# benfred/implicit

Hardware: AMD Instinct MI355X
Metric: ALS user+item updates/sec per iteration (factors=128); top-k recs/sec (higher is better)
Workload: dtype f32; 1 GPU; BASELINE configs[2]: last.fm-360K-shaped synthetic CSR, ALS CG cg_steps=3; users=358868, items=292385, nnz=17308340, factors=128, solver=cg, cg_steps=3

## Files before the change

### implicit_amd/csrc/als_cg_q.hip

```cpp
#include <type_traits>

#include "als_qtile.h"
#include "common.h"

namespace imp {

template <typename T>
void launch_team_fused(const imp_csr *C, int f, int width, int first, int count, T *X, const T *Y, const float *A0, int cg_steps,
                       const char *name);
template <typename T>
void launch_group_fused(const imp_csr *C, int f, int first, int count, T *X, const T *Y, const float *A0, int cg_steps, const char *name);
template <typename ST>
void launch_team_tile64(const imp_csr *C, int f, int width, int first, int count, ST *X, const ST *Y, const float *A0, int cg_steps,
                        const char *name);

template <int F, typename T> static void run_classes_q(const imp_csr *C, T *X, const T *Y, const float *A0, int cg_steps) {
  const int32_t *b = C->bin_start;
  constexpr bool kHalf = std::is_same<T, __half>::value;
  auto team = [&](int width32, int lo, int hi, const char *name) {
    if constexpr (kHalf) launch_team_tile64<T>(C, F, width32 / 2, lo, hi - lo, X, Y, A0, cg_steps, name);
    else launch_team_fused<T>(C, F, width32, lo, hi - lo, X, Y, A0, cg_steps, name);
  };
  team(16, b[1], b[2], "als_cg_team16_rows");
  team(8, b[2], b[3], "als_cg_team8_rows");
  team(4, b[3], b[4], "als_cg_team4_rows");
  team(2, b[4], b[5], "als_cg_team2_rows");
  if constexpr (F == 64) launch_team_fused<T>(C, F, 1, b[5], b[7] - b[5], X, Y, A0, cg_steps, "als_cg_short_rows");
  else launch_group_fused<T>(C, F, b[5], b[7] - b[5], X, Y, A0, cg_steps, "als_cg_short_rows");
}

template <typename T> void least_squares_cg_q(const imp_csr *C, T *X, const T *Y, const float *A0, int f, int cg_steps) {
  if (f == 128) run_classes_q<128, T>(C, X, Y, A0, cg_steps);
  else if (f == 64) run_classes_q<64, T>(C, X, Y, A0, cg_steps);
  else throw std::invalid_argument("least_squares_cg_q: f must be 64 or 128");
}
template void least_squares_cg_q<float>(const imp_csr *, float *, const float *, const float *, int, int);
template void least_squares_cg_q<__half>(const imp_csr *, __half *, const __half *, const float *, int, int);

}
```

### implicit_amd/csrc/als_cg_qf.hip

```cpp
#include <type_traits>

#include "als_qf_common.h"
#include "common.h"

namespace imp {

template <typename ST> struct Tile32 {
  typedef f32x2 elem;
  static constexpr int T = 32;
  static constexpr bool ROLL = std::is_same<ST, float>::value;
  static __device__ __forceinline__ void fetch(const int32_t *indices, const float *data, int lane, int k0, int end, int &col, float &c) {
    fetch_entries(indices, data, lane, k0, end, col, c);
  }
  template <int H> static __device__ __forceinline__ void gather(elem (&yq)[H], const ST *p) {
#pragma unroll
    for (int h = 0; h < H; h += 2) {
      const float4 v = load4(p + 32 * h);
      yq[h] = f32x2{v.x, v.y}, yq[h + 1] = f32x2{v.z, v.w};
    }
  }
  template <int H> static __device__ __forceinline__ float dot(const elem (&yq)[H], const f32x2 (&ve)[H]) {
    f32x2 s = yq[0] * ve[0];
#pragma unroll
    for (int h = 1; h < H; ++h) s = __builtin_elementwise_fma(yq[h], ve[h], s);
    return s.x + s.y;
  }
  template <int H> static __device__ __forceinline__ void axpy(const elem (&yq)[H], float w, f32x2 (&ae)[H]) {
    const f32x2 w2 = {w, w};
#pragma unroll
    for (int h = 0; h < H; ++h) ae[h] = __builtin_elementwise_fma(w2, yq[h], ae[h]);
  }
};

template <int F, int WPR, int BLOCK, typename ST>
__global__ __launch_bounds__(BLOCK, F == 64 ? 8 : 4) void als_cg_qfteam_kernel(const int32_t *__restrict__ order, int first, int count,
                                                                 const int32_t *__restrict__ indptr,
                                                                 const int32_t *__restrict__ indices,
                                                                 const float *__restrict__ data, ST *__restrict__ X,
                                                                 const ST *__restrict__ Y, const float *__restrict__ A0,
                                                                 int cg_steps) {
  team_rows<Tile32<ST>, F, WPR, BLOCK>(order, first, count, indptr, indices, data, X, Y, A0, cg_steps);
}

template <int F, int WPR, int BLOCK, typename T>
static void launch_qfteam(const imp_csr *C, int first, int count, T *X, const T *Y, const float *A0, int cg_steps,
                          const char *name) {
  if (count <= 0) return;
  constexpr int WAVES = BLOCK / 64, TEAMS = WAVES / WPR;
  size_t lds = team_lds_bytes<F, WPR, BLOCK, Tile32<T>::T>();
  auto kern = als_cg_qfteam_kernel<F, WPR, BLOCK, T>;
  IMP_CHECK_HIP(hipFuncSetAttribute(reinterpret_cast<const void *>(kern), hipFuncAttributeMaxDynamicSharedMemorySize, (int)lds));
  int per_cu = (int)std::max<size_t>(1, std::min<size_t>(2048 / BLOCK, (160 * 1024) / lds));
  constexpr int kBaseOversub = WPR <= 4 ? 4 : (WPR == 8 ? 2 : (F == 64 ? 2 : 1));
  int grid = std::min((count + TEAMS - 1) / TEAMS, ctx().num_cus * per_cu * std::max(kBaseOversub, ctx().oversub));
  IMP_PROF(name);
  kern<<<grid, BLOCK, lds, stream()>>>(C->order.data(), first, count, C->indptr.data(), C->indices.data(), C->data.data(), X, Y,
                                      A0, cg_steps);
  IMP_CHECK_HIP(hipGetLastError());
}

typedef float f32x4 __attribute__((ext_vector_type(4)));
template <int F> struct QFGroupCfg {
  static constexpr int LD = F + 8;
  static constexpr int LDB = F + 8;
  static constexpr int NT = F / 16;
  static constexpr int KH = 16 / NT;
  static constexpr int KB = (F / 16) / KH;
  static constexpr size_t lds_bytes = (size_t)3 * F * LDB * 2 + (size_t)3 * 16 * LDB * 2 +
                                      ((size_t)16 * LD + (size_t)KH * 16 * LD + 16 * 64) * sizeof(float);
};
typedef __bf16 bf16x8 __attribute__((ext_vector_type(8)));
typedef __bf16 bf16x2 __attribute__((ext_vector_type(2)));
__device__ __forceinline__ void split_bf16(float x, __bf16 &hi, __bf16 &mid, __bf16 &lo) {
  hi = (__bf16)x;
  const float r1 = x - (float)hi;
  mid = (__bf16)r1;
  lo = (__bf16)(r1 - (float)mid);
}

template <int F, bool FIRST, bool LAST, bool ROLL, typename ST>
__device__ __forceinline__ float tile_pass(f32x2 (&y)[8][F / 32], float *cw, int cnt, const float *vrow, float (&acc)[F / 64], int lane,
                                          int cnt_nx, int &col_nx, float &c_nx, const ST *__restrict__ Y) {
  using Tile = Tile32<ST>;
  constexpr int FE = F / 16, H = FE / 2;
  static_assert(!(FIRST && LAST) && (LAST || !ROLL), "pass form");
  if constexpr (ROLL) {
    col_nx = opaque(col_nx);
    c_nx = __int_as_float(opaque(__float_as_int(c_nx)));
  }
  f32x2 ve[H], ae[H];
  const float *cwg;
  {
// ... 295 lines not shown
```

### implicit_amd/csrc/als_qf_common.h

```cpp
#ifndef IMPLICIT_AMD_CSRC_ALS_QF_COMMON_H_
#define IMPLICIT_AMD_CSRC_ALS_QF_COMMON_H_
#include <type_traits>
#include <utility>

#include "als_qtile.h"

namespace imp {

__device__ __forceinline__ int opaque(int v) {
  asm volatile("" : "+v"(v));
  return v;
}

typedef float f32x2 __attribute__((ext_vector_type(2)));

template <int I> using idx_t = std::integral_constant<int, I>;
template <int N, typename Fn, int... Is> __device__ __forceinline__ void static_for_impl(Fn &&fn, std::integer_sequence<int, Is...>) {
  (fn(idx_t<Is>{}), ...);
}
template <int N, typename Fn> __device__ __forceinline__ void static_for(Fn &&fn) {
  static_for_impl<N>(fn, std::make_integer_sequence<int, N>{});
}

template <int F, int NJ, int TICKS> struct DenseTicks {
// ... 8 lines not shown
      if constexpr (NJ == 1) vj2 = f32x2{vp[0], 0.f};
      else if constexpr (s % 2 == 0) vj2 = *reinterpret_cast<const f32x2 *>(vp + s);
#pragma unroll
      for (int e = 0; e < Q4; ++e) a[e] = *reinterpret_cast<const float4 *>(row + (size_t)s * F + 64 * e);
    }
  }
  template <int K> __device__ __forceinline__ void consume(f32x2 (&ae)[FE / 2]) {
    if constexpr (K % EVERY == 0) {
      constexpr int s = K / EVERY;
      const float vj = (s % 2 == 0) ? vj2.x : vj2.y;
      const f32x2 v2 = {vj, vj};
#pragma unroll
      for (int e = 0; e < Q4; ++e) {
        ae[2 * e] = __builtin_elementwise_fma(v2, f32x2{a[e].x, a[e].y}, ae[2 * e]);
        ae[2 * e + 1] = __builtin_elementwise_fma(v2, f32x2{a[e].z, a[e].w}, ae[2 * e + 1]);
      }
    }
  }
};

__device__ __forceinline__ float reduce_pair(float d0, float d1) {
  float u = d1 + dpp_mov<0x128>(d1);
  const float s0 = d0 + dpp_mov<0x128>(d0);
  u = __builtin_bit_cast(float, __builtin_amdgcn_update_dpp(__builtin_bit_cast(int, u), __builtin_bit_cast(int, s0), 0xE4, 0xF, 0x3,
                                                            false));
  u += dpp_mov<0x141>(u);
  u += dpp_mov<0xB1>(u);
  u += dpp_mov<0x4E>(u);
  return u;
}
template <int LANE> __device__ __forceinline__ float row_bcast_from(float v) {
  return dpp_mov<0x150 + LANE>(v);
}

enum : unsigned { kGo = 1u, kLast = 2u };

#ifndef IMP_TEAM_NAP_FIRST
#define IMP_TEAM_NAP_FIRST 6
#endif
#ifndef IMP_TEAM_NAP_NEXT
#define IMP_TEAM_NAP_NEXT 2
#endif
#ifndef IMP_TEAM_NAP_LEADER
#define IMP_TEAM_NAP_LEADER 1
#endif
#ifndef IMP_TEAM_LEADER_PRIO
#define IMP_TEAM_LEADER_PRIO 0
#endif


template <typename Tile, int F, int P, typename ST>
__device__ __forceinline__ void gather_pair(typename Tile::elem (&y)[Tile::T / 4][F / 32], float *cw, int col_reg, float c_reg, int cnt,
                                            const ST *__restrict__ Y, int lane) {
  lane = opaque(lane);
  if ((lane >> 3) == P) {
    const bool ok = lane < cnt;
    cw[lane] = ok ? fabsf(c_reg) - 1.f : 0.f;
    cw[Tile::T + lane] = ok ? fmaxf(c_reg, 0.f) : 0.f;
  }
  const int src = 4 * (lane >> 4);
#pragma unroll
  for (int q = 2 * P; q < 2 * P + 2; ++q) {
    const unsigned col = (unsigned)__builtin_amdgcn_ds_bpermute(src + 16 * q, col_reg);
    Tile::template gather<F / 32>(y[q], Y + (size_t)col * F + 4 * (lane & 15));
  }
}
// ... 81 lines not shown
        dt.template issue<K>(row, vp);
        __builtin_amdgcn_sched_barrier(0);
        dt.template consume<K>(ae);
      });
    }
    if constexpr (ROLL) {
      if (8 * P < cnt_nx) gather_pair<Tile, F, P>(y, cw, col_nx, c_nx, cnt_nx, Y, lane);
    }
    __builtin_amdgcn_sched_barrier(0);
  });
  float pAp = 0.f;
  if constexpr (LAST) {
    f32x2 t = ae[0] * ve[0];
#pragma unroll
    for (int h = 1; h < H; ++h) t = __builtin_elementwise_fma(ae[h], ve[h], t);
    pAp = wave_allsum(fmaf(0.125f, s8, t.x + t.y));
  } else {
    float aes[FE];
#pragma unroll
    for (int h = 0; h < H; ++h) aes[2 * h] = ae[h].x, aes[2 * h + 1] = ae[h].y;
    reduce_expanded<F>(aes, acc);
  }
  if constexpr (ROLL) {
    Tile::fetch(indices, data, opaque(lane), k0_nx2, end_nx2, col_nx, c_nx);
  }
  return pAp;
}

template <int F, int WPR, int BLOCK, int T> constexpr size_t team_lds_bytes() {
  constexpr size_t WAVES = BLOCK / 64, TEAMS = WAVES / WPR;
  return ((size_t)F * F + WAVES * F + TEAMS * F + 2 * T * WAVES + 4 * TEAMS) * sizeof(float);
}

template <typename Tile, int F, int WPR, int BLOCK, typename ST>
__device__ __forceinline__ void team_rows(const int32_t *__restrict__ order, int first, int count, const int32_t *__restrict__ indptr,
                                          const int32_t *__restrict__ indices, const float *__restrict__ data, ST *__restrict__ X,
                                          const ST *__restrict__ Y, const float *__restrict__ A0, int cg_steps) {
  constexpr int FC = F / 64, FE = F / 16, T = Tile::T, WAVES = BLOCK / 64, TEAMS = WAVES / WPR, NJ = F / WPR / 4;
  static_assert(WPR <= WAVES && (F / WPR) % 4 == 0, "team width");
  extern __shared__ __attribute__((aligned(16))) float smem[];
  float *A0s = smem;
  float *parts = A0s + (size_t)F * F;
  float *vts = parts + (size_t)WAVES * F;
  float *cws = vts + (size_t)TEAMS * F;
  unsigned *ctl = reinterpret_cast<unsigned *>(cws + (size_t)WAVES * 2 * T);
  const int lane = threadIdx.x & 63;
  const int wave = __builtin_amdgcn_readfirstlane(threadIdx.x >> 6);
  const int team = wave / WPR, sub = wave % WPR;
  const bool leader = sub == 0;
  for (int e = threadIdx.x; e < F * F; e += BLOCK) A0s[e] = A0[e];
  if (threadIdx.x < 4 * TEAMS) ctl[threadIdx.x] = 0u;
  __syncthreads();
  const int j_begin = F * sub / WPR;
  float *vt = vts + (size_t)team * F;
  float *cw = cws + (size_t)wave * 2 * T;
  unsigned *arrivals = ctl + 4 * team, *generation = arrivals + 1, *words = arrivals + 2;

  unsigned gen = 0, pub = 0, arr_target = 0;
  auto lds_off = [](const void *ptr) { return (unsigned)(size_t)ptr; };
  const unsigned arrivals_off = lds_off(arrivals), generation_off = lds_off(generation), words_off = lds_off(words);
  const unsigned cf4 = 4u * (unsigned)QL<F>::cfactor(lane, 0);
  auto publish = [&](unsigned w) {
    ++pub;
    if (lane == 0)
      asm volatile("ds_write_b32 %0, %1\n\tds_add_u32 %2, %3" ::"v"(words_off + 4u * (pub & 1u)), "v"(w), "v"(generation_off), "v"(1u)
                   : "memory");
    if constexpr (IMP_TEAM_LEADER_PRIO > 0) __builtin_amdgcn_s_setprio(0);
  };
  auto poll = [&](unsigned off) {
    typedef __attribute__((address_space(3))) volatile unsigned lds_word;
    return (unsigned)__builtin_amdgcn_readfirstlane(*(lds_word *)(size_t)off);
  };
  auto await_operand = [&]() -> unsigned {
    ++gen;
    if constexpr (WPR > 1) {
      if (poll(generation_off) < gen) {
        __builtin_amdgcn_s_sleep(IMP_TEAM_NAP_FIRST);
        while (poll(generation_off) < gen) __builtin_amdgcn_s_sleep(IMP_TEAM_NAP_NEXT);
      }
    }
    return poll(words_off + 4u * (gen & 1u));
  };
  auto arrive = [&](const float (&acc)[FC]) {
// ... 31 lines not shown
    }
  };
  auto collect_scalar = [&](float own) -> float {
    arr_target += WPR;
    if constexpr (WPR > 1) {
      while (poll(arrivals_off) < arr_target) __builtin_amdgcn_s_sleep(IMP_TEAM_NAP_LEADER);
      asm volatile("" ::: "memory");
      if constexpr (IMP_TEAM_LEADER_PRIO > 0) __builtin_amdgcn_s_setprio(IMP_TEAM_LEADER_PRIO);
      const float *slot = parts + (size_t)(team * WPR) * F;
      float sum = 0.f;
#pragma unroll
      for (int w = 0; w < WPR; ++w) sum += slot[(size_t)w * F];
      return sum;
    } else {
      return own;
    }
  };
  auto operand_slot = [&]() { return reinterpret_cast<float *>(reinterpret_cast<char *>(vt) + cf4); };
  auto put_operand = [&](const float (&v)[FC]) {
    float *slot = operand_slot();
    if constexpr (FC == 2) *reinterpret_cast<float2 *>(slot) = make_float2(v[0], v[1]);
    else slot[0] = v[0];
  };
  auto get_operand = [&](float (&v)[FC]) {
    const float *slot = operand_slot();
    if constexpr (FC == 2) {
      const float2 t = *reinterpret_cast<const float2 *>(slot);
      v[0] = t.x, v[1] = t.y;
    } else {
      v[0] = slot[0];
    }
  };

  auto row_id = [&](int i) { return order[first + min(i, count - 1)]; };
  const int i_step = gridDim.x * TEAMS, i_first = blockIdx.x * TEAMS + team;
  auto slice = [&](int rb, int re, int &k0, int &cnt) {
    const int chunk = min(T, (((re - rb) + WPR - 1) / WPR + 3) & ~3);
    k0 = min(rb + chunk * sub, re);
    cnt = min(chunk, re - k0);
  };
  int id0 = row_id(i_first), id1 = row_id(i_first + i_step), id2 = row_id(i_first + 2 * i_step), id3 = row_id(i_first + 3 * i_step);
  int b0 = indptr[id0], e0 = indptr[id0 + 1], b1 = indptr[id1], e1 = indptr[id1 + 1], b2 = indptr[id2], e2 = indptr[id2 + 1];
  int ent_col, ent_cnt, k0;
  float ent_c;
  slice(b0, e0, k0, ent_cnt);
  Tile::fetch(indices, data, opaque(lane), k0, max(k0 + ent_cnt, b0 + 1), ent_col, ent_c);
  auto kill = [](float (&v)[FC]) {
#pragma unroll
    for (int cc = 0; cc < FC; ++cc) v[cc] = 0.f;
  };
  bool tile_ready = false;
  int cnt = 0;
  typename Tile::elem y[T / 4][FE / 2];
  float x[FC];
  kill(x);
  for (int i = i_first; i < count; i += i_step) {
    ST *xrow = X + (size_t)id0 * F;
    if (!tile_ready) {
      cnt = ent_cnt;
      ent_col = opaque(ent_col);
      ent_c = __int_as_float(opaque(__float_as_int(ent_c)));
      static_for<T / 8>([&](auto Pc) {
        constexpr int P = decltype(Pc)::value;
        if (8 * P < cnt) gather_pair<Tile, F, P>(y, cw, ent_col, ent_c, cnt, Y, lane);
      });
      slice(b1, e1, k0, ent_cnt);
      Tile::fetch(indices, data, opaque(lane), k0, max(k0 + ent_cnt, b1 + 1), ent_col, ent_c);
      if (leader) load_compact<F>(xrow, opaque(lane), x);
      else kill(x);
    }
    float xc[FC], r[FC], p[FC], Ap[FC], rsold = 0.f;
#pragma unroll
    for (int cc = 0; cc < FC; ++cc) xc[cc] = r[cc] = 0.f;
    bool store = false;
    if (leader) {
      put_operand(x);
#pragma unroll
      for (int cc = 0; cc < FC; ++cc) xc[cc] = x[cc];
      publish(kGo);
    }
    unsigned w = await_operand();
    {
      float acc[FC];
      fused_pass<Tile, F, NJ, true, false, false>(y, cw, cnt, vt, j_begin, A0s, acc, lane, 0, ent_col, ent_c, Y, nullptr, nullptr, 0, 0);
      arrive(acc);
    }
    if (leader) {
      collect(r);
#pragma unroll
      for (int cc = 0; cc < FC; ++cc) r[cc] = -r[cc], p[cc] = r[cc];
      rsold = dot_compact<F>(r, r);
      store = rsold >= 1e-20f;
      if (store && cg_steps > 0) {
        put_operand(p);
        publish(kGo | (cg_steps == 1 ? kLast : 0u));
      } else {
        publish(0u);
      }
    }
    w = await_operand();
    for (int it = 0; (w & (kGo | kLast)) == kGo; ++it) {
      float acc[FC];
      fused_pass<Tile, F, NJ, false, false, false>(y, cw, cnt, vt, j_begin, A0s, acc, lane, 0, ent_col, ent_c, Y, nullptr, nullptr, 0, 0);
      arrive(acc);
      if (leader) {
        collect(Ap);
        get_operand(p);
        const float alpha = rsold * __builtin_amdgcn_rcpf(dot_compact<F>(p, Ap));
#pragma unroll
        for (int cc = 0; cc < FC; ++cc) {
          xc[cc] = fmaf(alpha, p[cc], xc[cc]);
          r[cc] = fmaf(-alpha, Ap[cc], r[cc]);
        }
        const float rsnew = dot_compact<F>(r, r);
        if (rsnew < 1e-20f) {
          publish(0u);
        } else {
          const float beta = rsnew * __builtin_amdgcn_rcpf(rsold);
#pragma unroll
          for (int cc = 0; cc < FC; ++cc) p[cc] = fmaf(beta, p[cc], r[cc]);
          rsold = rsnew;
          put_operand(p);
          publish(kGo | (it + 2 >= cg_steps ? kLast : 0u));
        }
      }
      w = await_operand();
    }
    const bool rolled = Tile::ROLL && (w & kGo) != 0u;
    if (w & kGo) {
      float acc[FC], pAp;
      if constexpr (Tile::ROLL) {
        int k2, cnt2;
        slice(b2, e2, k2, cnt2);
        if (i + i_step >= count) ent_cnt = 0;
        pAp = fused_pass<Tile, F, NJ, false, true, true>(y, cw, cnt, vt, j_begin, A0s, acc, lane, ent_cnt, ent_col, ent_c, Y, indices,
                                                         data, k2, max(k2 + cnt2, b2 + 1));
        cnt = ent_cnt;
        ent_cnt = cnt2;
        if (leader) load_compact<F>(X + (size_t)id1 * F, opaque(lane), x);
        else kill(x);
      } else {
        kill(x);
        pAp = fused_pass<Tile, F, NJ, false, true, false>(y, cw, cnt, vt, j_begin, A0s, acc, lane, 0, ent_col, ent_c, Y, nullptr,
                                                          nullptr, 0, 0);
      }
      arrive_scalar(pAp);
      if (leader) {
        pAp = collect_scalar(pAp);
        get_operand(p);
        const float alpha = rsold * __builtin_amdgcn_rcpf(pAp);
#pragma unroll
        for (int cc = 0; cc < FC; ++cc) xc[cc] = fmaf(alpha, p[cc], xc[cc]);
        publish(0u);
      }
      (void)await_operand();
    } else {
      kill(x);
    }
    if (leader && store) store_compact<F>(xrow, opaque(lane), xc);
    tile_ready = rolled;
    id0 = id1, id1 = id2, id2 = id3, id3 = row_id(i + 4 * i_step);
    b0 = b1, e0 = e1, b1 = b2, e1 = e2, b2 = indptr[id2], e2 = indptr[id2 + 1];
  }
}

}
#endif
```

### implicit_amd/csrc/common.h

```cpp
#ifndef IMPLICIT_AMD_CSRC_COMMON_H_
#define IMPLICIT_AMD_CSRC_COMMON_H_

#include <hip/hip_runtime.h>

#include <climits>
#include <cstdint>
#include <cstdio>
#include <memory>
#include <mutex>
#include <stdexcept>
#include <string>
#include <vector>

#include "../../include/implicit_hip.h"
#include "csr_schedule.h"

namespace imp {

struct out_of_range_error : std::runtime_error {
  using std::runtime_error::runtime_error;
};

void set_last_error(const std::string &msg);

#define IMP_CHECK_HIP(expr)                                                                    \
  do {                                                                                         \
    hipError_t _e = (expr);                                                                    \
    if (_e != hipSuccess) {                                                                    \
      throw std::runtime_error(std::string("HIP error: ") + hipGetErrorString(_e) + " (" +    \
                               __FILE__ + ":" + std::to_string(__LINE__) + ")");             \
    }                                                                                          \
  } while (0)

struct Context;
Context &ctx();
std::unique_lock<std::recursive_mutex> lock_device();

template <typename F> int guarded(F &&body) {
  try {
    auto lock = lock_device();
    body();
    return IMP_OK;
  } catch (const std::invalid_argument &e) {
    set_last_error(e.what());
    return IMP_INVALID_ARGUMENT;
  } catch (const out_of_range_error &e) {
    set_last_error(e.what());
    return IMP_OUT_OF_RANGE;
// ... 15 lines not shown
    return IMP_INVALID_ARGUMENT;
  } catch (const out_of_range_error &e) {
    set_last_error(e.what());
    return IMP_OUT_OF_RANGE;
  } catch (const std::exception &e) {
    set_last_error(e.what());
    return IMP_RUNTIME_ERROR;
  } catch (...) {
    set_last_error("unknown error");
    return IMP_RUNTIME_ERROR;
  }
}

inline hipStream_t stream();
void sync();
void sync_call();
unsigned long long *fixup_total();
struct SolverSwitches {
  bool nm;
  bool w256;
  bool cg_pad;
  bool chol_nm;
  bool chol_pad;
};
const SolverSwitches &solver_switches();

struct ProfScope {
  explicit ProfScope(const char *name);
  ~ProfScope();
  const char *name;
  hipEvent_t start = nullptr, stop = nullptr;
};
bool prof_enabled();
#define IMP_PROF(name) ::imp::ProfScope _prof_scope_(name)

struct Context;
struct Storage {
  void *ptr = nullptr;
  size_t bytes = 0;
  bool owned = true;
  Context *home = nullptr;
  int size_class = -1;
  bool exposed = false;
  static constexpr size_t kSmallMax = (size_t)4 << 20;
  Storage(size_t bytes_, bool zero);
  Storage(void *foreign) : ptr(foreign), owned(false) {}
  ~Storage();
  Storage(const Storage &) = delete;
  Storage &operator=(const Storage &) = delete;
};

template <typename T> struct DeviceArray {
  std::shared_ptr<Storage> storage;
  size_t size = 0;
  T *data() const { return storage ? reinterpret_cast<T *>(storage->ptr) : nullptr; }
  void alloc(size_t n, bool zero = false) {
    storage = std::make_shared<Storage>(n * sizeof(T), zero);
    size = n;
  }
  void upload(const T *host, size_t n) {
    alloc(n);
    if (n) IMP_CHECK_HIP(hipMemcpyAsync(data(), host, n * sizeof(T), hipMemcpyHostToDevice, stream()));
  }
};

struct PaddedSystem {
// ... 5 lines not shown
  void forget_y() { y_src = nullptr; }
  bool y_made_from(const void *dst, size_t bytes) const {
    const char *a = static_cast<const char *>(dst), *b = static_cast<const char *>(y_src);
    return b && a < b + y_rows * (size_t)y_f * sizeof(float) && b < a + bytes;
  }
  void release() {
    x = {}, y = {}, gram = {};
    forget_y();
  }
};

struct Context {
  int device = 0;
  hipStream_t stream = nullptr;
  int num_cus = 256;
  int oversub = 1;
  bool deferred = false;
  hipStream_t occupy_stream = nullptr;
  std::recursive_mutex mutex;
  std::mutex small_mutex;
  std::vector<void *> small_free[24];
  void *pin_stage = nullptr;
  size_t pin_stage_bytes = 0;
  hipEvent_t pin_stage_ev = nullptr;
  DeviceArray<float> gram_ws;
  DeviceArray<float> long_ws;
  PaddedSystem pad;
  DeviceArray<double> loss_buf;
  DeviceArray<unsigned long long> chol_failed;
  DeviceArray<float> barrier_word;
  unsigned long long *fixup_total = nullptr;
  DeviceArray<float> w256_ws;
  DeviceArray<unsigned> nm_fix_rows;
  DeviceArray<int> nm_ticket;
  DeviceArray<unsigned long long> bpr_stats;
  DeviceArray<float> lmf_ws;
  DeviceArray<double> knn_acc;
  DeviceArray<int32_t> knn_touched;
  int knn_cols = -1;
};
inline hipStream_t stream() { return ctx().stream; }
void note_device_write(const void *dst, size_t bytes);
struct DerivedCache {
  const void *src = nullptr;
  size_t bytes = 0;
};
void register_derived_cache(DerivedCache *c);
void unregister_derived_cache(DerivedCache *c);

}

struct imp_matrix {
  size_t rows = 0, cols = 0, itemsize = 4;
  void *data = nullptr;
  std::shared_ptr<imp::Storage> storage;
  size_t bytes() const { return rows * cols * itemsize; }
  float *f32() const {
    if (itemsize != 4) throw std::runtime_error("can't cast Matrix to float*");
    return reinterpret_cast<float *>(data);
  }
};

struct imp_intvector {
  imp::DeviceArray<int32_t> v;
  size_t size = 0;
};
// ... 76 lines not shown
```

### implicit_amd/csrc/containers.hip

```cpp
#include <hip/hip_fp16.h>

#include <algorithm>
#include <cstring>
#include <map>
#include <mutex>
#include <thread>

#include "common.h"

namespace imp {

static thread_local std::string g_last_error;
void set_last_error(const std::string &msg) { g_last_error = msg; }

static std::mutex g_ctx_mutex;
static auto &g_contexts = *new std::map<int, std::unique_ptr<Context>>;

Context &ctx() {
  int dev = 0;
  IMP_CHECK_HIP(hipGetDevice(&dev));
  std::lock_guard<std::mutex> lock(g_ctx_mutex);
  auto it = g_contexts.find(dev);
  if (it == g_contexts.end()) {
    auto c = std::make_unique<Context>();
// ... 47 lines not shown
  static const SolverSwitches s = [] {
    SolverSwitches v;
    v.nm = env_unless_zero("IMP_NM");
    v.w256 = getenv("IMP_F256_OLD") == nullptr;
    v.cg_pad = getenv("IMP_NO_PAD") == nullptr;
    v.chol_nm = env_unless_zero("IMP_CHOL_NM");
    v.chol_pad = v.chol_nm && env_unless_zero("IMP_CHOL_PAD");
    return v;
  }();
  return s;
}

void sync() { IMP_CHECK_HIP(hipStreamSynchronize(stream())); }
void sync_call() {
  if (!ctx().deferred) sync();
}

struct ProfEntry {
  double total_ms = 0;
  int64_t launches = 0;
};
struct ProfPending {
  const char *name;
  hipEvent_t start, stop;
};
static std::recursive_mutex g_prof_mutex;
static bool g_prof_on = false;
static std::string g_prof_filter;
static std::map<std::string, ProfEntry> g_prof;
static std::vector<ProfPending> g_prof_pending;
static std::vector<hipEvent_t> g_event_pool;

bool prof_enabled() { return g_prof_on; }

static hipEvent_t get_event() {
  if (!g_event_pool.empty()) {
    hipEvent_t e = g_event_pool.back();
    g_event_pool.pop_back();
    return e;
  }
  hipEvent_t e;
  IMP_CHECK_HIP(hipEventCreate(&e));
  return e;
}

static void prof_account(const ProfPending &p) {
  float ms = 0;
  if (hipEventElapsedTime(&ms, p.start, p.stop) == hipSuccess) {
    auto &e = g_prof[p.name];
    e.total_ms += ms;
    e.launches += 1;
  }
  g_event_pool.push_back(p.start);
  g_event_pool.push_back(p.stop);
}

static void prof_collect_finished() {
  size_t done = 0;
  while (done < g_prof_pending.size() && hipEventQuery(g_prof_pending[done].stop) == hipSuccess) prof_account(g_prof_pending[done++]);
  if (done) g_prof_pending.erase(g_prof_pending.begin(), g_prof_pending.begin() + (long)done);
}

ProfScope::ProfScope(const char *n) : name(n) {
  if (!g_prof_on) return;
  std::lock_guard<std::recursive_mutex> plock(g_prof_mutex);
  if (!g_prof_filter.empty() && !strstr(n, g_prof_filter.c_str())) return;
// ... 363 lines not shown
          t_data[at] = data[k];
        }
    });
  });
}

int imp_host_csr_plan(int32_t rows, int32_t cols, const int32_t *indptr, const int32_t *indices, int32_t segment, int32_t stripe,
                      int32_t nm_segment, int32_t num_cus, int which, int32_t *order, int32_t *bin_start, int32_t *row_seg,
                      int64_t seg_capacity, int32_t *seg_row, int32_t *seg_begin, int32_t *seg_end, int32_t *seg_exec,
                      int32_t *xcd_start, int32_t *info) {
  return guarded_host([&] {
    if (which < 0 || which > 2) throw std::invalid_argument("host_csr_plan: which must be 0 (all), 1 (chol) or 2 (nm)");
    if (nm_segment < 0) throw std::invalid_argument("host_csr_plan: nm_segment must be positive, or 0 for the automatic length");
    if (rows < 0) throw std::invalid_argument("negative dimension for CSRMatrix");
    validate_csr(rows, cols, rows ? (int64_t)indptr[rows] : 0, indptr, indices);
    PlanKnobs knobs;
    knobs.segment = segment, knobs.stripe = stripe, knobs.nm_segment = nm_segment, knobs.num_cus = num_cus;
    const HostSchedule s = plan_csr(rows, cols, indptr, indices, knobs);
    const HostPlan &p = which == 0 ? s.plan_all : which == 1 ? s.plan_chol : s.plan_nm;
    if (p.n_seg > seg_capacity) throw std::invalid_argument("host_csr_plan: the plan has more segments than seg_capacity");
    std::copy(s.order.begin(), s.order.end(), order);
    std::copy(s.bin_start, s.bin_start + imp_csr::kBins + 1, bin_start);
    std::copy(p.row_seg.begin(), p.row_seg.end(), row_seg);
    std::copy(p.seg_row.begin(), p.seg_row.end(), seg_row);
    std::copy(p.seg_begin.begin(), p.seg_begin.end(), seg_begin);
    std::copy(p.seg_end.begin(), p.seg_end.end(), seg_end);
    std::copy(p.seg_exec.begin(), p.seg_exec.end(), seg_exec);
    std::copy(p.xcd_start, p.xcd_start + 9, xcd_start);
    const int32_t fields[8] = {p.n_long, p.n_seg, p.striped, s.n_chol_long, s.nm_segment, s.nm_multi_rows, s.nm_multi_segs, 0};
    std::copy(fields, fields + 8, info);
  });
}

int imp_matrix_create(size_t rows, size_t cols, const void *host_data, size_t itemsize, imp_matrix **out) {
  return guarded([&] {
    imp_matrix *m = new_matrix(rows, cols, itemsize, host_data == nullptr);
    std::unique_ptr<imp_matrix> guard(m);
    if (host_data && m->bytes()) {
      IMP_CHECK_HIP(hipMemcpyAsync(m->data, host_data, m->bytes(), hipMemcpyHostToDevice, stream()));
    }
    sync();
    *out = guard.release();
  });
}

int imp_matrix_wrap_device(size_t rows, size_t cols, void *device_ptr, size_t itemsize, imp_matrix **out) {
  return guarded([&] {
    if (itemsize != 4 && itemsize != 2) throw std::invalid_argument("invalid itemsize for Matrix (must be 2 or 4)");
    auto m = std::make_unique<imp_matrix>();
    m->rows = rows;
    m->cols = cols;
    m->itemsize = itemsize;
    m->storage = std::make_shared<Storage>(device_ptr);
    m->data = device_ptr;
    *out = m.release();
  });
}

int imp_matrix_row(const imp_matrix *src, size_t rowid, imp_matrix **out) {
  return guarded([&] {
    if (rowid >= src->rows) throw std::invalid_argument("row index out of bounds for matrix");
    auto m = std::make_unique<imp_matrix>(*src);
    m->rows = 1;
    m->data = reinterpret_cast<char *>(src->data) + rowid * src->cols * src->itemsize;
    *out = m.release();
  });
// ... 373 lines not shown
```

### implicit_amd/gpu/_hip.py

```python
import ctypes
import os

_HERE = os.path.dirname(os.path.abspath(__file__))
from .. import _libpath

LIB_PATH = _libpath.OVERRIDE or os.path.join(os.path.dirname(_HERE), "libimplicit_hip.so")

c_void_pp = ctypes.POINTER(ctypes.c_void_p)
c_i32_p = ctypes.POINTER(ctypes.c_int32)
c_f32_p = ctypes.POINTER(ctypes.c_float)

IMP_OK, IMP_INVALID_ARGUMENT, IMP_OUT_OF_RANGE, IMP_RUNTIME_ERROR = 0, 1, 2, 3

_SIGNATURES = {
    "imp_get_device_count": [ctypes.POINTER(ctypes.c_int)],
    "imp_set_device": [ctypes.c_int],
    "imp_get_device": [ctypes.POINTER(ctypes.c_int)],
    "imp_set_oversubscribe": [ctypes.c_int],
    "imp_get_oversubscribe": [ctypes.POINTER(ctypes.c_int)],
    "imp_set_deferred_sync": [ctypes.c_int],
    "imp_debug_occupy": [ctypes.c_int, ctypes.c_int],
    "imp_debug_core_clock": [ctypes.c_int, ctypes.POINTER(ctypes.c_double)],
    "imp_device_synchronize": [],
    "imp_solver_fixup_rows": [ctypes.POINTER(ctypes.c_ulonglong), ctypes.c_int],
    "imp_mem_get_info": [ctypes.POINTER(ctypes.c_size_t), ctypes.POINTER(ctypes.c_size_t)],
    "imp_release_workspaces": [],
    "imp_host_csr_transpose": [ctypes.c_int32, ctypes.c_int32, ctypes.c_int64, ctypes.c_void_p, ctypes.c_void_p, ctypes.c_void_p,
                               ctypes.c_void_p, ctypes.c_void_p, ctypes.c_void_p, ctypes.c_int],
    "imp_host_csr_plan": [ctypes.c_int32, ctypes.c_int32, ctypes.c_void_p, ctypes.c_void_p, ctypes.c_int32, ctypes.c_int32,
                          ctypes.c_int32, ctypes.c_int32, ctypes.c_int, ctypes.c_void_p, ctypes.c_void_p, ctypes.c_void_p,
                          ctypes.c_int64, ctypes.c_void_p, ctypes.c_void_p, ctypes.c_void_p, ctypes.c_void_p, ctypes.c_void_p,
                          ctypes.c_void_p],
    "imp_matrix_create": [ctypes.c_size_t, ctypes.c_size_t, ctypes.c_void_p, ctypes.c_size_t, c_void_pp],
    "imp_matrix_wrap_device": [ctypes.c_size_t, ctypes.c_size_t, ctypes.c_void_p, ctypes.c_size_t, c_void_pp],
    "imp_matrix_row": [ctypes.c_void_p, ctypes.c_size_t, c_void_pp],
    "imp_matrix_slice": [ctypes.c_void_p, ctypes.c_size_t, ctypes.c_size_t, c_void_pp],
    "imp_matrix_gather": [ctypes.c_void_p, ctypes.c_void_p, c_void_pp],
    "imp_matrix_resize": [ctypes.c_void_p, ctypes.c_size_t, ctypes.c_size_t],
    "imp_matrix_assign_rows": [ctypes.c_void_p, ctypes.c_void_p, ctypes.c_void_p],
    "imp_matrix_astype": [ctypes.c_void_p, ctypes.c_size_t, c_void_pp],
    "imp_matrix_calculate_norms": [ctypes.c_void_p, c_void_pp],
    "imp_matrix_to_host": [ctypes.c_void_p, ctypes.c_void_p],
    "imp_matrix_from_host": [ctypes.c_void_p, ctypes.c_void_p],
    "imp_matrix_copy_rows": [ctypes.c_void_p, ctypes.c_size_t, ctypes.c_void_p, ctypes.c_size_t, ctypes.c_size_t],
    "imp_matrix_shape": [ctypes.c_void_p, ctypes.POINTER(ctypes.c_size_t), ctypes.POINTER(ctypes.c_size_t),
                         ctypes.POINTER(ctypes.c_size_t)],
    "imp_matrix_device_ptr": [ctypes.c_void_p, c_void_pp],
    "imp_matrix_destroy": [ctypes.c_void_p],
    "imp_intvector_create": [ctypes.c_void_p, ctypes.c_size_t, c_void_pp],
    "imp_intvector_destroy": [ctypes.c_void_p],
    "imp_csr_create": [ctypes.c_int32, ctypes.c_int32, ctypes.c_int64, ctypes.c_void_p, ctypes.c_void_p,
                       ctypes.c_void_p, c_void_pp],
    "imp_csr_create64": [ctypes.c_int32, ctypes.c_int32, ctypes.c_int64, ctypes.c_void_p, ctypes.c_void_p,
                         ctypes.c_void_p, c_void_pp],
    "imp_csr_shape": [ctypes.c_void_p, c_i32_p, c_i32_p, ctypes.POINTER(ctypes.c_int64)],
    "imp_csr_destroy": [ctypes.c_void_p],
    "imp_coo_create": [ctypes.c_int32, ctypes.c_int32, ctypes.c_int64, ctypes.c_void_p, ctypes.c_void_p,
                       ctypes.c_void_p, c_void_pp],
    "imp_coo_create_from_csr_pattern": [ctypes.c_int32, ctypes.c_int32, ctypes.c_void_p, ctypes.c_int, ctypes.c_void_p,
                                        ctypes.POINTER(ctypes.c_void_p)],
    "imp_coo_destroy": [ctypes.c_void_p],
    "imp_solver_create": [c_void_pp],
    "imp_solver_destroy": [ctypes.c_void_p],
    "imp_solver_calculate_yty": [ctypes.c_void_p, ctypes.c_void_p, ctypes.c_void_p, ctypes.c_float],
    "imp_solver_least_squares": [ctypes.c_void_p, ctypes.c_void_p, ctypes.c_void_p, ctypes.c_void_p,
# ... 80 lines not shown
```

### implicit_amd/utils.py

```python
import time
import warnings

import numpy as np
import scipy.sparse


class ParameterWarning(Warning):
    """Raised (as a warning) when an input had to be converted (implicit/utils.py:155-156)."""


def check_csr(user_items):
    if isinstance(user_items, scipy.sparse.csr_matrix):
        return user_items
    kind = type(user_items).__name__
    t0 = time.time()
    converted = user_items.tocsr()
    warnings.warn(
        f"Method expects CSR input, and was passed {kind} instead. "
        f"Converting to CSR took {time.time() - t0} seconds",
        ParameterWarning,
    )
    return converted


# ... 53 lines not shown
    indptr, indices, data = (np.ascontiguousarray(a) for a in (m.indptr, m.indices, m.data))
    t_indptr = np.empty(cols + 1, dtype=np.int32)
    t_indices = np.empty(m.nnz, dtype=np.int32)
    t_data = np.empty(m.nnz, dtype=np.float32)
    check(fn(rows, cols, m.nnz, indptr.ctypes.data, indices.ctypes.data, data.ctypes.data, t_indptr.ctypes.data,
             t_indices.ctypes.data, t_data.ctypes.data, int(threads)))
    out = scipy.sparse.csr_matrix((t_data, t_indices, t_indptr), shape=(cols, rows), copy=False)
    out.has_sorted_indices = True
    out.has_canonical_format = True
    return out


def csr_schedule(m, which=0, segment=512, stripe=-1, nm_segment=0, num_cus=256):
    from .gpu._hip import check, lib

    rows, cols = m.shape
    indptr = np.ascontiguousarray(m.indptr, dtype=np.int32)
    indices = np.ascontiguousarray(m.indices, dtype=np.int32)
    capacity = max(int(indptr[-1]), 0) if rows else 0
    out = {"order": np.empty(rows, np.int32), "bin_start": np.empty(9, np.int32), "row_seg": np.empty(rows + 1, np.int32)}
    segs = {k: np.empty(capacity, np.int32) for k in ("seg_row", "seg_begin", "seg_end", "seg_exec")}
    out["xcd_start"] = np.empty(9, np.int32)
    info = np.zeros(8, np.int32)
    check(lib().imp_host_csr_plan(rows, cols, indptr.ctypes.data, indices.ctypes.data, segment, stripe, nm_segment, num_cus, which,
                                  out["order"].ctypes.data, out["bin_start"].ctypes.data, out["row_seg"].ctypes.data, capacity,
                                  *(segs[k].ctypes.data for k in ("seg_row", "seg_begin", "seg_end", "seg_exec")),
                                  out["xcd_start"].ctypes.data, info.ctypes.data))
    names = ("n_long", "n_seg", "striped", "n_chol_long", "nm_segment", "nm_multi_rows", "nm_multi_segs")
    out.update({k: int(v) for k, v in zip(names, info)})
    out["striped"] = bool(out["striped"])
    out["row_seg"] = out["row_seg"][:out["n_long"] + 1]
    out.update({k: v[:out["n_seg"]] for k, v in segs.items()})
    return out
```

### include/implicit_hip.h

```cpp
#ifndef IMPLICIT_HIP_H_
#define IMPLICIT_HIP_H_

#include <stddef.h>
#include <stdint.h>

#ifdef __cplusplus
extern "C" {
#endif

typedef enum {
  IMP_OK = 0,
  IMP_INVALID_ARGUMENT = 1,
  IMP_OUT_OF_RANGE = 2,
  IMP_RUNTIME_ERROR = 3
} imp_status;

typedef struct imp_matrix imp_matrix;
typedef struct imp_intvector imp_intvector;
typedef struct imp_csr imp_csr;
typedef struct imp_coo imp_coo;
typedef struct imp_solver imp_solver;
typedef struct imp_knn imp_knn;
typedef struct imp_random imp_random;
typedef struct imp_comm imp_comm;

const char *imp_last_error(void);
int imp_get_device_count(int *count);
int imp_set_device(int device);
int imp_get_device(int *device);
int imp_set_oversubscribe(int factor);
int imp_get_oversubscribe(int *factor);
int imp_set_deferred_sync(int on);
int imp_debug_occupy(int workgroups, int microseconds);
int imp_debug_core_clock(int microseconds, double *mhz);
int imp_device_synchronize(void);
int imp_solver_fixup_rows(unsigned long long *count, int reset);
int imp_mem_get_info(size_t *free_bytes, size_t *total_bytes);
int imp_release_workspaces(void);
const char *imp_version(void);

int imp_host_csr_transpose(int32_t rows, int32_t cols, int64_t nonzeros, const int32_t *indptr, const int32_t *indices,
                           const float *data, int32_t *t_indptr, int32_t *t_indices, float *t_data, int threads);

int imp_host_csr_plan(int32_t rows, int32_t cols, const int32_t *indptr, const int32_t *indices, int32_t segment, int32_t stripe,
                      int32_t nm_segment, int32_t num_cus, int which, int32_t *order, int32_t *bin_start, int32_t *row_seg,
                      int64_t seg_capacity, int32_t *seg_row, int32_t *seg_begin, int32_t *seg_end, int32_t *seg_exec,
                      int32_t *xcd_start, int32_t *info);

int imp_matrix_create(size_t rows, size_t cols, const void *host_data, size_t itemsize, imp_matrix **out);
int imp_matrix_wrap_device(size_t rows, size_t cols, void *device_ptr, size_t itemsize, imp_matrix **out);
int imp_matrix_row(const imp_matrix *m, size_t rowid, imp_matrix **out);
int imp_matrix_slice(const imp_matrix *m, size_t start, size_t end, imp_matrix **out);
int imp_matrix_gather(const imp_matrix *m, const imp_intvector *rowids, imp_matrix **out);
int imp_matrix_resize(imp_matrix *m, size_t rows, size_t cols);
int imp_matrix_assign_rows(imp_matrix *m, const imp_intvector *rowids, const imp_matrix *other);
int imp_matrix_astype(const imp_matrix *m, size_t itemsize, imp_matrix **out);
int imp_matrix_calculate_norms(const imp_matrix *m, imp_matrix **out);
int imp_matrix_to_host(const imp_matrix *m, void *host_out);
int imp_matrix_from_host(imp_matrix *m, const void *host_in);
int imp_matrix_copy_rows(imp_matrix *dst, size_t dst_row, const imp_matrix *src, size_t src_row, size_t rows);
int imp_matrix_shape(const imp_matrix *m, size_t *rows, size_t *cols, size_t *itemsize);
int imp_matrix_device_ptr(const imp_matrix *m, void **ptr);
int imp_matrix_destroy(imp_matrix *m);

int imp_intvector_create(const int32_t *host_data, size_t size, imp_intvector **out);
int imp_intvector_destroy(imp_intvector *v);
int imp_csr_create(int32_t rows, int32_t cols, int64_t nonzeros, const int32_t *indptr,
                   const int32_t *indices, const float *data, imp_csr **out);
int imp_csr_create64(int32_t rows, int32_t cols, int64_t nonzeros, const int64_t *indptr,
                     const int32_t *indices, const float *data, imp_csr **out);
int imp_csr_shape(const imp_csr *m, int32_t *rows, int32_t *cols, int64_t *nonzeros);
int imp_csr_destroy(imp_csr *m);
int imp_coo_create(int32_t rows, int32_t cols, int64_t nonzeros, const int32_t *row,
                   const int32_t *col, const float *data, imp_coo **out);
int imp_coo_create_from_csr_pattern(int32_t rows, int32_t cols, const void *indptr, int indptr_is_64,
                                    const int32_t *indices, imp_coo **out);
int imp_coo_destroy(imp_coo *m);

int imp_solver_create(imp_solver **out);
int imp_solver_destroy(imp_solver *s);
// ... 58 lines not shown
```

Baseline: 164.6 million updates/s.

## Chain team8/4/2 CG classes into one persistent kernel with atomic ticket scheduling

For fp32 storage at F=128, the three separate team launches (width 8, 4, 2) are replaced by one persistent chain kernel. It stages the Gramian once and walks the classes in sequence. Within each class, rows are handed out dynamically by atomic counters split over eight queues, not by a static grid stride. The per-launch ticket bases are tracked on the host so the counters never need resetting. This is meant to cut launch overhead and tail imbalance between classes, at the cost of atomic traffic, a more complex stop protocol, and a single LDS size fixed to the largest class.

```diff
diff --git a/implicit_amd/csrc/als_cg_q.hip b/implicit_amd/csrc/als_cg_q.hip
--- a/implicit_amd/csrc/als_cg_q.hip
+++ b/implicit_amd/csrc/als_cg_q.hip
@@ -14,6 +14,10 @@
 void launch_team_tile64(const imp_csr *C, int f, int width, int first, int count, ST *X, const ST *Y, const float *A0, int cg_steps,
                         const char *name);
 
+template <typename T>
+void launch_team_chain(const imp_csr *C, int f, const int (&first)[3], const int (&count)[3], T *X, const T *Y, const float *A0, int cg_steps,
+                       const char *name);
+
 template <int F, typename T> static void run_classes_q(const imp_csr *C, T *X, const T *Y, const float *A0, int cg_steps) {
   const int32_t *b = C->bin_start;
   constexpr bool kHalf = std::is_same<T, __half>::value;
@@ -22,9 +26,14 @@
     else launch_team_fused<T>(C, F, width32, lo, hi - lo, X, Y, A0, cg_steps, name);
   };
   team(16, b[1], b[2], "als_cg_team16_rows");
-  team(8, b[2], b[3], "als_cg_team8_rows");
-  team(4, b[3], b[4], "als_cg_team4_rows");
-  team(2, b[4], b[5], "als_cg_team2_rows");
+  if (F == 128 && !kHalf && !prof_unfiltered()) {
+    const int first[3] = {b[2], b[3], b[4]}, count[3] = {b[3] - b[2], b[4] - b[3], b[5] - b[4]};
+    launch_team_chain<T>(C, F, first, count, X, Y, A0, cg_steps, "als_cg_team_chain_rows");
+  } else {
+    team(8, b[2], b[3], "als_cg_team8_rows");
+    team(4, b[3], b[4], "als_cg_team4_rows");
+    team(2, b[4], b[5], "als_cg_team2_rows");
+  }
   if constexpr (F == 64) launch_team_fused<T>(C, F, 1, b[5], b[7] - b[5], X, Y, A0, cg_steps, "als_cg_short_rows");
   else launch_group_fused<T>(C, F, b[5], b[7] - b[5], X, Y, A0, cg_steps, "als_cg_short_rows");
 }
diff --git a/implicit_amd/csrc/als_cg_qf.hip b/implicit_amd/csrc/als_cg_qf.hip
--- a/implicit_amd/csrc/als_cg_qf.hip
+++ b/implicit_amd/csrc/als_cg_qf.hip
@@ -1,4 +1,6 @@
 #include <type_traits>
+
+#include <algorithm>
 
 #include "als_qf_common.h"
 #include "common.h"
@@ -58,6 +60,78 @@
                                       A0, cg_steps);
   IMP_CHECK_HIP(hipGetLastError());
 }
+
+struct ChainClassArgs {
+  int first[ChainTickets::kClasses], count[ChainTickets::kClasses];
+  unsigned base[ChainTickets::kClasses][ChainTickets::kQueues];
+};
+static_assert(ChainTickets::kQueues == kTicketQueues, "queues of a ticketed class");
+template <int F> constexpr size_t chain_lds_bytes() {
+  return std::max(team_lds_bytes<F, 8, 512, 32>(), std::max(team_lds_bytes<F, 4, 512, 32>(), team_lds_bytes<F, 2, 512, 32>()));
+}
+template <int F, typename ST>
+__global__ __launch_bounds__(512, F == 64 ? 8 : 4) void als_cg_qfteam_chain_kernel(const int32_t *__restrict__ order, ChainClassArgs cls,
+                                                                                  unsigned *__restrict__ counters,
+                                                                                  const int32_t *__restrict__ indptr,
+                                                                                  const int32_t *__restrict__ indices,
+                                                                                  const float *__restrict__ data, ST *__restrict__ X,
+                                                                                  const ST *__restrict__ Y, const float *__restrict__ A0,
+                                                                                  int cg_steps) {
+  static_assert(Tile32<ST>::T == 32, "chain_lds_bytes");
+  team_stage_gramian<F, 512>(A0);
+  bool entered = false;
+  static_for<ChainTickets::kClasses>([&](auto Cc) {
+    constexpr int C = decltype(Cc)::value, WPR = 8 >> C;
+    if (cls.count[C] > 0) {
+      if (entered) __syncthreads();
+      entered = true;
+      team_rows<Tile32<ST>, F, WPR, 512, true, false>(order, cls.first[C], cls.count[C], indptr, indices, data, X, Y, A0, cg_steps,
+                                                      counters + (C * kTicketQueues + blockIdx.x % kTicketQueues) * ChainTickets::kCounterStride,
+                                                      cls.base[C][blockIdx.x % kTicketQueues]);
+    }
+  });
+}
+
+static int team512_per_cu(size_t lds) { return (int)std::max<size_t>(1, std::min<size_t>(2048 / 512, (160 * 1024) / lds)); }
+
+template <typename T>
+void launch_team_chain(const imp_csr *C, int f, const int (&first)[3], const int (&count)[3], T *X, const T *Y, const float *A0, int cg_steps,
+                       const char *name) {
+  if constexpr (std::is_same<T, float>::value) {
+    auto run = [&](auto Fc) {
+      constexpr int F = decltype(Fc)::value;
+      if (count[0] <= 0 && count[1] <= 0 && count[2] <= 0) return;
+      const size_t lds = chain_lds_bytes<F>();
+      auto kern = als_cg_qfteam_chain_kernel<F, T>;
+      IMP_CHECK_HIP(hipFuncSetAttribute(reinterpret_cast<const void *>(kern), hipFuncAttributeMaxDynamicSharedMemorySize, (int)lds));
+      const int grid = std::max(ctx().num_cus * team512_per_cu(lds), ChainTickets::kQueues);
+      ChainClassArgs cls;
+      const int teams[3] = {1, 2, 4};
+      for (int c = 0; c < 3; ++c) {
+        if (count[c] >= ChainTickets::kMaxCount) throw std::invalid_argument("launch_team_chain: too many rows in a class");
+        cls.first[c] = first[c], cls.count[c] = std::max(count[c], 0);
+      }
+      Context &cx = ctx();
+      if (!cx.chain_counters.data())
+        cx.chain_counters.alloc((size_t)ChainTickets::kClasses * ChainTickets::kQueues * ChainTickets::kCounterStride, true);
+      ChainTickets after = cx.chain_tickets;
+      after.launch(cls.count, grid, teams, cls.base);
+      IMP_PROF(name);
+      kern<<<grid, 512, lds, stream()>>>(C->order.data(), cls, cx.chain_counters.data(), C->indptr.data(), C->indices.data(),
+                                        C->data.data(), X, Y, A0, cg_steps);
+      IMP_CHECK_HIP(hipGetLastError());
+      cx.chain_tickets = after;
+    };
+    if (f == 128) run(idx_t<128>{});
+    else throw std::invalid_argument("launch_team_chain: f must be 128");
+  } else {
+    throw std::invalid_argument("launch_team_chain: fp32 storage only (float16 storage runs its classes on the packed tiles)");
+  }
+}
+template void launch_team_chain<float>(const imp_csr *, int, const int (&)[3], const int (&)[3], float *, const float *, const float *, int,
+                                       const char *);
+template void launch_team_chain<__half>(const imp_csr *, int, const int (&)[3], const int (&)[3], __half *, const __half *, const float *,
+                                        int, const char *);
 
 typedef float f32x4 __attribute__((ext_vector_type(4)));
 template <int F> struct QFGroupCfg {
diff --git a/implicit_amd/csrc/als_qf_common.h b/implicit_amd/csrc/als_qf_common.h
--- a/implicit_amd/csrc/als_qf_common.h
+++ b/implicit_amd/csrc/als_qf_common.h
@@ -64,6 +64,8 @@
 template <int LANE> __device__ __forceinline__ float row_bcast_from(float v) {
   return dpp_mov<0x150 + LANE>(v);
 }
+
+constexpr int kTicketQueues = 8;
 
 enum : unsigned { kGo = 1u, kLast = 2u };
 
@@ -211,12 +213,19 @@
   return ((size_t)F * F + WAVES * F + TEAMS * F + 2 * T * WAVES + 4 * TEAMS) * sizeof(float);
 }
 
-template <typename Tile, int F, int WPR, int BLOCK, typename ST>
+template <int F, int BLOCK> __device__ __forceinline__ void team_stage_gramian(const float *__restrict__ A0) {
+  extern __shared__ __attribute__((aligned(16))) float smem[];
+  for (int e = threadIdx.x; e < F * F; e += BLOCK) smem[e] = A0[e];
+}
+
+template <typename Tile, int F, int WPR, int BLOCK, bool TICKETS = false, bool STAGE = true, typename ST>
 __device__ __forceinline__ void team_rows(const int32_t *__restrict__ order, int first, int count, const int32_t *__restrict__ indptr,
                                           const int32_t *__restrict__ indices, const float *__restrict__ data, ST *__restrict__ X,
-                                          const ST *__restrict__ Y, const float *__restrict__ A0, int cg_steps) {
+                                          const ST *__restrict__ Y, const float *__restrict__ A0, int cg_steps,
+                                          unsigned *counter = nullptr, unsigned base = 0u) {
   constexpr int FC = F / 64, FE = F / 16, T = Tile::T, WAVES = BLOCK / 64, TEAMS = WAVES / WPR, NJ = F / WPR / 4;
   static_assert(WPR <= WAVES && (F / WPR) % 4 == 0, "team width");
+  static_assert(!TICKETS || WPR > 1, "tickets travel in the team protocol");
   extern __shared__ __attribute__((aligned(16))) float smem[];
   float *A0s = smem;
   float *parts = A0s + (size_t)F * F;
@@ -227,7 +236,9 @@
   const int wave = __builtin_amdgcn_readfirstlane(threadIdx.x >> 6);
   const int team = wave / WPR, sub = wave % WPR;
   const bool leader = sub == 0;
-  for (int e = threadIdx.x; e < F * F; e += BLOCK) A0s[e] = A0[e];
+  if constexpr (STAGE) {
+    for (int e = threadIdx.x; e < F * F; e += BLOCK) A0s[e] = A0[e];
+  }
   if (threadIdx.x < 4 * TEAMS) ctl[threadIdx.x] = 0u;
   __syncthreads();
   const int j_begin = F * sub / WPR;
@@ -325,8 +336,23 @@
     }
   };
 
-  auto row_id = [&](int i) { return order[first + min(i, count - 1)]; };
-  const int i_step = gridDim.x * TEAMS, i_first = blockIdx.x * TEAMS + team;
+  const int queue = TICKETS ? (int)(blockIdx.x % kTicketQueues) : 0;
+  const int rows = TICKETS ? (count - queue + kTicketQueues - 1) / kTicketQueues : count;
+  auto row_id = [&](int i) {
+    return order[first + min(TICKETS ? kTicketQueues * i + queue : i, count - 1)];
+  };
+  const int i_step = TICKETS ? (int)((gridDim.x - queue + kTicketQueues - 1) / kTicketQueues) * TEAMS : gridDim.x * TEAMS;
+  const int i_first = TICKETS ? (int)(blockIdx.x / kTicketQueues) * TEAMS + team : blockIdx.x * TEAMS + team;
+  int t1 = i_first + i_step, t2 = i_first + 2 * i_step, t3 = i_first + 3 * i_step;
+  unsigned drawn_ticket = (unsigned)rows, drawn = 0u;
+  auto draw = [&]() {
+    if (lane == 0) asm volatile("global_atomic_add %0, %1, %2, off sc0" : "=v"(drawn) : "v"(counter), "v"(1u) : "memory");
+  };
+  auto take_draw = [&]() {
+    asm volatile("s_waitcnt vmcnt(0)" : "+v"(drawn)::"memory");
+    drawn_ticket = min((unsigned)__builtin_amdgcn_readfirstlane(drawn) - base + 4u * (unsigned)i_step, (unsigned)rows);
+  };
+  auto stop_word = [&]() -> unsigned { return TICKETS ? drawn_ticket << 2 : 0u; };
   auto slice = [&](int rb, int re, int &k0, int &cnt) {
     const int chunk = min(T, (((re - rb) + WPR - 1) / WPR + 3) & ~3);
     k0 = min(rb + chunk * sub, re);
@@ -347,7 +373,7 @@
   typename Tile::elem y[T / 4][FE / 2];
   float x[FC];
   kill(x);
-  for (int i = i_first; i < count; i += i_step) {
+  for (int i = i_first; i < rows; i += TICKETS ? 0 : i_step) {
     ST *xrow = X + (size_t)id0 * F;
     if (!tile_ready) {
       cnt = ent_cnt;
@@ -371,6 +397,9 @@
 #pragma unroll
       for (int cc = 0; cc < FC; ++cc) xc[cc] = x[cc];
       publish(kGo);
+      if constexpr (TICKETS) {
+        if (t3 < rows) draw();
+      }
     }
     unsigned w = await_operand();
     {
@@ -384,11 +413,14 @@
       for (int cc = 0; cc < FC; ++cc) r[cc] = -r[cc], p[cc] = r[cc];
       rsold = dot_compact<F>(r, r);
       store = rsold >= 1e-20f;
+      if constexpr (TICKETS) {
+        if (t3 < rows) take_draw();
+      }
       if (store && cg_steps > 0) {
         put_operand(p);
         publish(kGo | (cg_steps == 1 ? kLast : 0u));
       } else {
-        publish(0u);
+        publish(stop_word());
       }
     }
     w = await_operand();
@@ -407,7 +439,7 @@
         }
         const float rsnew = dot_compact<F>(r, r);
         if (rsnew < 1e-20f) {
-          publish(0u);
+          publish(stop_word());
         } else {
           const float beta = rsnew * __builtin_amdgcn_rcpf(rsold);
 #pragma unroll
@@ -425,7 +457,7 @@
       if constexpr (Tile::ROLL) {
         int k2, cnt2;
         slice(b2, e2, k2, cnt2);
-        if (i + i_step >= count) ent_cnt = 0;
+        if ((TICKETS ? t1 : i + i_step) >= rows) ent_cnt = 0;
         pAp = fused_pass<Tile, F, NJ, false, true, true>(y, cw, cnt, vt, j_begin, A0s, acc, lane, ent_cnt, ent_col, ent_c, Y, indices,
                                                          data, k2, max(k2 + cnt2, b2 + 1));
         cnt = ent_cnt;
@@ -444,15 +476,21 @@
         const float alpha = rsold * __builtin_amdgcn_rcpf(pAp);
 #pragma unroll
         for (int cc = 0; cc < FC; ++cc) xc[cc] = fmaf(alpha, p[cc], xc[cc]);
-        publish(0u);
-      }
-      (void)await_operand();
+        publish(stop_word());
+      }
+      if constexpr (TICKETS) w = await_operand();
+      else (void)await_operand();
     } else {
       kill(x);
     }
     if (leader && store) store_compact<F>(xrow, opaque(lane), xc);
     tile_ready = rolled;
-    id0 = id1, id1 = id2, id2 = id3, id3 = row_id(i + 4 * i_step);
+    if constexpr (TICKETS) {
+      i = t1, t1 = t2, t2 = t3, t3 = (int)(w >> 2);
+      id0 = id1, id1 = id2, id2 = id3, id3 = row_id(t3);
+    } else {
+      id0 = id1, id1 = id2, id2 = id3, id3 = row_id(i + 4 * i_step);
+    }
     b0 = b1, e0 = e1, b1 = b2, e1 = e2, b2 = indptr[id2], e2 = indptr[id2 + 1];
   }
 }
diff --git a/implicit_amd/csrc/common.h b/implicit_amd/csrc/common.h
--- a/implicit_amd/csrc/common.h
+++ b/implicit_amd/csrc/common.h
@@ -14,6 +14,7 @@
 
 #include "../../include/implicit_hip.h"
 #include "csr_schedule.h"
+#include "team_tickets.h"
 
 namespace imp {
 
@@ -95,6 +96,7 @@
   hipEvent_t start = nullptr, stop = nullptr;
 };
 bool prof_enabled();
+bool prof_unfiltered();
 #define IMP_PROF(name) ::imp::ProfScope _prof_scope_(name)
 
 struct Context;
@@ -166,6 +168,8 @@
   unsigned long long *fixup_total = nullptr;
   DeviceArray<float> w256_ws;
   DeviceArray<unsigned> nm_fix_rows;
+  DeviceArray<unsigned> chain_counters;
+  ChainTickets chain_tickets;
   DeviceArray<int> nm_ticket;
   DeviceArray<unsigned long long> bpr_stats;
   DeviceArray<float> lmf_ws;
diff --git a/implicit_amd/csrc/containers.hip b/implicit_amd/csrc/containers.hip
--- a/implicit_amd/csrc/containers.hip
+++ b/implicit_amd/csrc/containers.hip
@@ -103,6 +103,10 @@
 static std::vector<hipEvent_t> g_event_pool;
 
 bool prof_enabled() { return g_prof_on; }
+bool prof_unfiltered() {
+  std::lock_guard<std::recursive_mutex> plock(g_prof_mutex);
+  return g_prof_on && g_prof_filter.empty();
+}
 
 static hipEvent_t get_event() {
   if (!g_event_pool.empty()) {
@@ -532,6 +536,29 @@
   });
 }
 
+int imp_host_chain_tickets(uint32_t *next, const int32_t *count, int32_t workgroups, const int32_t *teams_per_workgroup, uint32_t *base,
+                           uint32_t *draws) {
+  return guarded_host([&] {
+    constexpr int NC = ChainTickets::kClasses, NQ = ChainTickets::kQueues;
+    ChainTickets t;
+    int32_t c[NC], n[NC];
+    uint32_t b[NC][NQ];
+    if (workgroups <= 0) throw std::invalid_argument("host_chain_tickets: the grid holds at least one workgroup");
+    for (int k = 0; k < NC; ++k) {
+      if (count[k] < 0 || count[k] >= ChainTickets::kMaxCount || teams_per_workgroup[k] <= 0)
+        throw std::invalid_argument("host_chain_tickets: a class holds 0 .. 2^30 - 1 rows and a workgroup at least one team");
+      c[k] = count[k], n[k] = teams_per_workgroup[k];
+      for (int q = 0; q < NQ; ++q) t.next[k][q] = next[k * NQ + q];
+    }
+    t.launch(c, workgroups, n, b);
+    for (int k = 0; k < NC; ++k)
+      for (int q = 0; q < NQ; ++q) {
+        draws[k * NQ + q] = t.next[k][q] - next[k * NQ + q];
+        next[k * NQ + q] = t.next[k][q], base[k * NQ + q] = b[k][q];
+      }
+  });
+}
+
 int imp_matrix_create(size_t rows, size_t cols, const void *host_data, size_t itemsize, imp_matrix **out) {
   return guarded([&] {
     imp_matrix *m = new_matrix(rows, cols, itemsize, host_data == nullptr);
diff --git a/implicit_amd/csrc/team_tickets.h b/implicit_amd/csrc/team_tickets.h
--- /dev/null
+++ b/implicit_amd/csrc/team_tickets.h
@@ -0,0 +1,37 @@
+#ifndef IMPLICIT_AMD_CSRC_TEAM_TICKETS_H_
+#define IMPLICIT_AMD_CSRC_TEAM_TICKETS_H_
+
+#include <algorithm>
+#include <cstdint>
+
+namespace imp {
+
+struct ChainTickets {
+  static constexpr int kClasses = 3;
+  static constexpr int kQueues = 8;
+  static constexpr int kCounterStride = 64;
+  static constexpr int32_t kMaxCount = 1 << 30;
+  uint32_t next[kClasses][kQueues] = {};
+
+  static int32_t queue_rows(int32_t count, int q) { return count > q ? (count - q + kQueues - 1) / kQueues : 0; }
+  static int32_t queue_workgroups(int32_t workgroups, int q) { return queue_rows(workgroups, q); }
+  static uint32_t draws(int32_t count, int32_t teams) {
+    if (count <= 0 || teams <= 0) return 0u;
+    const int64_t n = teams, c = count;
+    const int64_t inside = std::max<int64_t>(0, c - 4 * n);
+    const int64_t past = std::min<int64_t>(n, std::max<int64_t>(0, c - 3 * n));
+    return (uint32_t)(inside + past);
+  }
+  void launch(const int32_t (&count)[kClasses], int32_t workgroups, const int32_t (&teams_per_workgroup)[kClasses],
+              uint32_t (&base)[kClasses][kQueues]) {
+    for (int c = 0; c < kClasses; ++c)
+      for (int q = 0; q < kQueues; ++q) {
+        base[c][q] = next[c][q];
+        next[c][q] += draws(queue_rows(count[c], q), queue_workgroups(workgroups, q) * teams_per_workgroup[c]);
+      }
+  }
+};
+
+}
+
+#endif
diff --git a/implicit_amd/gpu/_hip.py b/implicit_amd/gpu/_hip.py
--- a/implicit_amd/gpu/_hip.py
+++ b/implicit_amd/gpu/_hip.py
@@ -31,6 +31,7 @@
                           ctypes.c_int32, ctypes.c_int32, ctypes.c_int, ctypes.c_void_p, ctypes.c_void_p, ctypes.c_void_p,
                           ctypes.c_int64, ctypes.c_void_p, ctypes.c_void_p, ctypes.c_void_p, ctypes.c_void_p, ctypes.c_void_p,
                           ctypes.c_void_p],
+    "imp_host_chain_tickets": [ctypes.c_void_p, ctypes.c_void_p, ctypes.c_int32, ctypes.c_void_p, ctypes.c_void_p, ctypes.c_void_p],
     "imp_matrix_create": [ctypes.c_size_t, ctypes.c_size_t, ctypes.c_void_p, ctypes.c_size_t, c_void_pp],
     "imp_matrix_wrap_device": [ctypes.c_size_t, ctypes.c_size_t, ctypes.c_void_p, ctypes.c_size_t, c_void_pp],
     "imp_matrix_row": [ctypes.c_void_p, ctypes.c_size_t, c_void_pp],
diff --git a/implicit_amd/utils.py b/implicit_amd/utils.py
--- a/implicit_amd/utils.py
+++ b/implicit_amd/utils.py
@@ -109,3 +109,16 @@
     out["row_seg"] = out["row_seg"][:out["n_long"] + 1]
     out.update({k: v[:out["n_seg"]] for k, v in segs.items()})
     return out
+
+
+def chain_tickets(state, counts, workgroups, teams_per_workgroup=(1, 2, 4)):
+    from .gpu._hip import check, lib
+
+    assert state.dtype == np.uint32 and state.shape == (3, 8) and state.flags.c_contiguous
+    counts = np.ascontiguousarray(counts, dtype=np.int32)
+    teams = np.ascontiguousarray(teams_per_workgroup, dtype=np.int32)
+    assert counts.shape == teams.shape == (3,)
+    base, draws = np.empty((3, 8), np.uint32), np.empty((3, 8), np.uint32)
+    check(lib().imp_host_chain_tickets(state.ctypes.data, counts.ctypes.data, int(workgroups), teams.ctypes.data, base.ctypes.data,
+                                       draws.ctypes.data))
+    return base, draws
diff --git a/include/implicit_hip.h b/include/implicit_hip.h
--- a/include/implicit_hip.h
+++ b/include/implicit_hip.h
@@ -46,6 +46,9 @@
                       int32_t nm_segment, int32_t num_cus, int which, int32_t *order, int32_t *bin_start, int32_t *row_seg,
                       int64_t seg_capacity, int32_t *seg_row, int32_t *seg_begin, int32_t *seg_end, int32_t *seg_exec,
                       int32_t *xcd_start, int32_t *info);
+
+int imp_host_chain_tickets(uint32_t *next, const int32_t *count, int32_t workgroups, const int32_t *teams_per_workgroup, uint32_t *base,
+                           uint32_t *draws);
 
 int imp_matrix_create(size_t rows, size_t cols, const void *host_data, size_t itemsize, imp_matrix **out);
 int imp_matrix_wrap_device(size_t rows, size_t cols, void *device_ptr, size_t itemsize, imp_matrix **out);
```

Result: faster. 171.3 million updates/s (median of 6 runs) (+4.1%).
